# csiro-robotics/syropod_highlevel_controller

Measured on AMD Instinct MI355X. Metric: control-cycles/sec (all legs IK-solved), higher is better.
Workload: dtype f64

## Files before the change

syropod_highlevel_controller_amd/csrc/shc_cycle.hpp:

```cpp
#pragma once

#include "../../include/shc_batch.h"
#include "shc_leg.hpp"

namespace shc {

enum : int { WS_STARTING = 0, WS_MOVING = 1, WS_STOPPING = 2, WS_STOPPED = 3 };
enum : int { SS_SWING = 0, SS_STANCE = 1, SS_FORCE_STANCE = 2, SS_FORCE_STOP = 3 };
enum : int { PS_POSING = 0, PS_STOP_POSING = 1, PS_POSING_COMPLETE = 2 };
enum : int { PM_NONE = 0, PM_SWING = 1, PM_STANCE = 2, PM_STOP = 3 };

constexpr int LW_ACP = 1 << 2, LW_CFS = 1 << 3, LW_PM_SHIFT = 4, LW_NEG = 1 << 6, LW_IKFAIL = 1 << 7, LW_PHASE_SHIFT = 8,
              LW_PHASE_MASK = 0xFFFFF, LW_ZBV = 1 << 28, LW_ATT = 1 << 29, LW_ROTDEF = 1 << 30,
              LW_TARGROT = int(1u << 31);
constexpr int RW_LACP_SHIFT = 2, RW_LCFS_SHIFT = 6, RW_RTDA = 1 << 10, RW_APS_SHIFT = 11;

constexpr int kMaxAutoPosers = 8;
constexpr int kSwingTable = 64;
enum : unsigned { DIRTY_WALK_PLANE = 1, DIRTY_MANUAL = 2, DIRTY_SWING_ORG = 4, DIRTY_STANCE_ORG = 8,
                  DIRTY_TARG_DIR = 16,
                  DIRTY_LAST = DIRTY_TARG_DIR };
enum : unsigned { RT_MANUAL_LIVE = 1, RT_TOUCHDOWN = 2, RT_EXTERNAL = 4, RT_MANUAL_LEGS = 8, RT_EFFORT_LIVE = 16, RT_SKIP_MARKED = 32, RT_POSE_MARKED = 64 };

enum : unsigned { F_MANUAL = 1, F_AUTO = 2, F_INCL = 4, F_IMU = 8, F_ADM = 16, F_TIPF = 32, F_ODOM = 64, F_DYN = 1u << 31,
// ... 118 lines not shown
};
SHC_HD double set_precision3(double v) { return round_to_int(v * 1000.0) / 1000.0; }
SHC_HD double stance_span_change_y(const double *table, int leg, double default_shift_z) {
  const double *t = table + leg * SpanTable::kStride;
  const int n = int(t[0]);
  const double target = set_precision3(default_shift_z);
  int lower = -1, upper = -1;
  for (int k = 0; k < n; ++k) {
    const double h = t[2 + 2 * k];
    if (h > target && (upper < 0 || h < t[2 + 2 * upper])) upper = k;
    if (h <= target && (lower < 0 || h > t[2 + 2 * lower])) lower = k;
  }
  if (lower < 0 || upper < 0) return 0.0;
  const double uh = set_precision3(t[2 + 2 * upper]), lh = set_precision3(t[2 + 2 * lower]);
  const double i = (target - lh) / (uh - lh);
  const double radius = t[3 + 2 * lower] * (1.0 - i) + t[3 + 2 * upper] * i;
  return radius * t[1];
}

#if defined(__HIPCC__)

template <int L, int NJ, unsigned F>
constexpr bool phase_fences() {
#if defined(SHC_FENCE)
  return true;
#else
  constexpr bool exact = (F & (0x80000000u  | 0x40000000u )) == 0;
  constexpr bool octo_tipf = L == 8 && NJ == 5 && (F & 32u ) != 0 && (F & 16u ) == 0;
  return exact && ((NJ == 4 && (L == 4 || L == 8)) || octo_tipf);
#endif
}
#define SHC_PHASE_FENCE() do { if constexpr (phase_fences<L, NJ, F>()) __builtin_amdgcn_sched_barrier(0); } while (0)
#if defined(SHC_RES2_TIMING) && !defined(SHC_RES2_BUSY_ONLY)
__shared__ long long shc_ticks_lds[96];
__shared__ long long shc_acc_lds[96];
#define SHC_TICK(i) do { __builtin_amdgcn_sched_barrier(0); if (blockIdx.x == 1 && (threadIdx.x & 127) == 0) shc_ticks_lds[(threadIdx.x >> 7) * 32 + (i)] = __builtin_readcyclecounter(); __builtin_amdgcn_sched_barrier(0); } while (0)
#else
#define SHC_TICK(i) do {} while (0)
#endif
#ifdef SHC_ABLATE
#define SHC_DBG(P) ((P).debug_skip)
#else
#define SHC_DBG(P) 0
#endif
__device__ __forceinline__ int uni(int v) { return __builtin_amdgcn_readfirstlane(v); }

template <unsigned F>
struct Feat {
  __device__ __forceinline__ static bool manual(const CycleParams &P) { return (F & F_DYN) ? P.manual_posing != 0 : (F & F_MANUAL) != 0; }
  __device__ __forceinline__ static bool autop(const CycleParams &P) { return (F & F_DYN) ? P.auto_posing != 0 : (F & F_AUTO) != 0; }
  __device__ __forceinline__ static bool incl(const CycleParams &P) { return (F & F_DYN) ? P.inclination_posing != 0 : (F & F_INCL) != 0; }
  __device__ __forceinline__ static bool imu(const CycleParams &P) { return (F & F_DYN) ? P.imu_posing != 0 : (F & F_IMU) != 0; }
  __device__ __forceinline__ static bool adm(const CycleParams &P) { return (F & F_DYN) ? P.admittance_control != 0 : (F & F_ADM) != 0; }
  __device__ __forceinline__ static bool tipf(const CycleParams &P) { return (F & F_DYN) ? P.tip_force != 0 : (F & F_TIPF) != 0; }
  __device__ __forceinline__ static bool odom(const CycleParams &P) { return (F & F_DYN) ? P.odometry != 0 : (F & F_ODOM) != 0; }
};

template <int L>
struct Group {
  int base;
  __device__ __forceinline__ int get(int v, int j) const { return __shfl(v, base + j, 64); }
  __device__ __forceinline__ double get(double v, int j) const { return __shfl(v, base + j, 64); }
  __device__ __forceinline__ double sum(double v) const {
    double s = 0.0;
#pragma unroll
    for (int j = 0; j < L; ++j) s += get(v, j);
    return s;
  }
// ... 1444 lines not shown
```

syropod_highlevel_controller_amd/csrc/shc_cycle_inst.hip:

```cpp
#include "shc_cycle_kernel.hpp"
#include "shc_cycle_select.hpp"

#if !defined(SHC_INST_L) || !defined(SHC_INST_NJ) || !defined(SHC_INST_PART)
#error "compile with -DSHC_INST_L=<legs> -DSHC_INST_NJ=<joints> -DSHC_INST_PART=<0|1>"
#endif

#include <cstdio>
#include <cstdlib>
#include <mutex>
#include <set>
#include <tuple>

namespace shc {

static void note_kernel(const char *form, int legs, int joints, unsigned features) {
  static const char *path = std::getenv("SHC_KERNEL_LOG");
  if (!path) return;
  static std::mutex mu;
  static std::set<std::tuple<const char *, unsigned>> seen;
  std::lock_guard<std::mutex> lock(mu);
  if (!seen.insert({form, features}).second) return;
  if (FILE *f = std::fopen(path, "a")) {
    std::fprintf(f, "%s %d %d %u\n", form, legs, joints, features);
    std::fclose(f);
  }
}

template <int L, int NJ, unsigned F>
static void launch_cycle(const CycleLaunch &a) {
  constexpr int RPW = 64 / L;
  constexpr size_t wave_bytes = size_t(RobotFields::COUNT * RPW + PK_COUNT * 64 + (RobotFields::I_COUNT * RPW + 1) / 2) * 8;
#if SHC_INST_PART == 1
  if (a.fit) {
    a.fit->supported = has_resident(F) ? 1 : 0;
    a.fit->batch = has_batch(F) ? 1 : 0;
    a.fit->two_wave = has_two_wave(F) ? 1 : 0;
    a.fit->helper_wave = has_helper_wave(L, NJ, F) ? 1 : 0;
    a.fit->blocks_per_cu = 0;
    if constexpr (has_resident(F)) {
      int blocks = 0;
      if (hipOccupancyMaxActiveBlocksPerMultiprocessor(&blocks, shc_resident_kernel<L, NJ, F>, 64, wave_bytes) != hipSuccess) blocks = 0;
      a.fit->blocks_per_cu = blocks;
    }
  } else if (a.resident->batch_cycles != 0) {
    if constexpr (has_batch(F)) {
      note_kernel("batch", L, NJ, F);
      shc_batch_kernel<L, NJ, F><<<dim3(a.grid), dim3(a.block), wave_bytes * (a.block / 64), a.stream>>>(a.st, (const SharedConsts<L, NJ> *)a.consts, *a.resident, a.rt_flags);
    }
  } else if (a.block == 384) {
    if constexpr (has_helper_wave(L, NJ, F)) {
      static_assert(has_two_wave(F), "the three-role form is a form of the two-wavefront pipeline");
      note_kernel("resident3", L, NJ, F);
      shc_resident2_kernel<L, NJ, F, true><<<dim3(a.grid), dim3(384), 2 * wave_bytes + sizeof(Resident3Lds<L, NJ>), a.stream>>>(
          a.st, (const SharedConsts<L, NJ> *)a.consts, *a.resident, a.rt_flags);
    }
  } else if (a.block == 256) {
    if constexpr (has_two_wave(F)) {
      note_kernel("resident2", L, NJ, F);
      shc_resident2_kernel<L, NJ, F><<<dim3(a.grid), dim3(256), 2 * wave_bytes + sizeof(Resident2Lds<L, NJ>), a.stream>>>(
          a.st, (const SharedConsts<L, NJ> *)a.consts, *a.resident, a.rt_flags);
    }
  } else {
    if constexpr (has_resident(F)) {
      note_kernel("resident", L, NJ, F);
      shc_resident_kernel<L, NJ, F><<<dim3(a.grid), dim3(64), wave_bytes, a.stream>>>(a.st, (const SharedConsts<L, NJ> *)a.consts, *a.resident, a.rt_flags);
    }
  }
#else
  if constexpr (has_half_kernels(F)) {
    const int64_t waves = int64_t(a.grid) * (a.block / 64);
    if (a.half_steps >= 0 && (a.half_steps > 0 || waves >= 2048)) {
      note_kernel("half", L, NJ, F);
      for (int c = 0; c < a.n_cycles; ++c) {
        shc_cycle_half_kernel<L, NJ, F, ROLE_FRONT><<<dim3(a.grid), dim3(a.block), wave_bytes * (a.block / 64), a.stream>>>(
            a.st, (const SharedConsts<L, NJ> *)a.consts, a.rt_flags, a.wave0);
        shc_cycle_half_kernel<L, NJ, F, ROLE_BACK><<<dim3(a.grid), dim3(a.block), wave_bytes * (a.block / 64), a.stream>>>(
            a.st, (const SharedConsts<L, NJ> *)a.consts, a.rt_flags, a.wave0);
      }
      return;
    }
  }
  note_kernel("cycle", L, NJ, F);
  shc_cycle_kernel<L, NJ, F><<<dim3(a.grid), dim3(a.block), wave_bytes * (a.block / 64), a.stream>>>(a.st, (const SharedConsts<L, NJ> *)a.consts, a.n_cycles,
                                                                                              a.rt_flags, a.wave0);
#endif
}
// ... 22 lines not shown
```

syropod_highlevel_controller_amd/csrc/shc_cycle_kernel.hpp:

```cpp
#pragma once

#include "shc_cycle.hpp"
#include "shc_cycle_launch.hpp"

#include <hip/hip_runtime.h>

#include <type_traits>

namespace shc {

#ifndef SHC_WAVES_PER_SIMD
#define SHC_WAVES_PER_SIMD 2
#endif
#ifndef SHC_ROT_WAVES_PER_SIMD
#define SHC_ROT_WAVES_PER_SIMD 1
#endif
#ifndef SHC_TERRAIN_WAVES_PER_SIMD
#define SHC_TERRAIN_WAVES_PER_SIMD 2
#endif

struct LegPlanes {
  double2 *base;
  int64_t ns;
  uint32_t slot;
// ... 900 lines not shown
      if (t0 == 0) t0 = now;
      else if (now - t0 > 1000 * ticks_per_ms) {
        *fault = true;
        return true;
      }
    }
    return false;
  }
  __device__ __forceinline__ void operator()() const {
    volatile unsigned *flag = flag_at;
    unsigned spins = 0;
    u64 t0 = 0;
    while (*flag != want)
      if (give_up(spins, t0)) break;
    __builtin_amdgcn_fence(__ATOMIC_ACQUIRE, "workgroup");
  }
};
template <int L, int NJ>
struct Resident2Lds {
  double mailbox[2][2][13][64];
  double pose_c[2][2][64];
  unsigned pose_done[2];
  unsigned model_dirty[2], model_seen[2], model_fault[2];
  double stiff[2][64];
  int ikfail[2][64];
  unsigned long long ctrl[4][4];
};
template <int L, int NJ>
struct Resident3Lds : Resident2Lds<L, NJ> {
  int leg_word[2][2][64];
  unsigned back_seen[2];
  double tip_xy[2][2][2][64];
  unsigned front_done[2];
};

template <int L, int NJ, unsigned F, bool HELPER = false>
__global__ void __launch_bounds__(HELPER ? 384 : 256, 1) shc_resident2_kernel(DevState st, const SharedConsts<L, NJ> *gc, ResidentArgs A, unsigned rt_flags) {
  using R = RobotFields;
  using FD = Fields<NJ>;
  using FT = Feat<F>;
  constexpr int RPW = 64 / L;
  constexpr int kThreads = HELPER ? 384 : 256;
  if (blockIdx.x == 0) {
    if (threadIdx.x < 64) resident_relay<PART_GATE>(A);
    else if (threadIdx.x < 128) resident_relay<PART_DONE>(A);
    return;
  }
  __shared__ SharedConsts<L, NJ> C;
  extern __shared__ double wave_lds[];
  constexpr int kWaveDoubles = R::COUNT * RPW + PK_COUNT * 64 + (R::I_COUNT * RPW + 1) / 2;
  using Lds = std::conditional_t<HELPER, Resident3Lds<L, NJ>, Resident2Lds<L, NJ>>;
  Lds &X = *reinterpret_cast<Lds *>(wave_lds + 2 * kWaveDoubles);
  const bool manual_live = (rt_flags & RT_MANUAL_LIVE) != 0;
  const int lane = threadIdx.x & 63;
  const int wib = __builtin_amdgcn_readfirstlane(threadIdx.x >> 6);
  const int pair = wib & 1;
  const bool walker = wib < 2, helper = HELPER && wib >= 4, leader = wib == (HELPER ? 4 : 2);
  const int64_t wave = (int64_t(blockIdx.x) - 1) * 2 + pair;
  const bool active = wave < A.n_waves;
  const int64_t rob0 = wave * RPW;
  const int64_t left = st.n_robots - rob0;
  const int robots_here = !active ? 0 : (left < RPW ? (left < 0 ? 0 : int(left)) : RPW);
  int grp = lane / L;
  const int leg = lane - grp * L;
  const bool live = grp < robots_here;
  if (grp >= robots_here) grp = robots_here > 0 ? robots_here - 1 : 0;
  const uint32_t slot = uint32_t((active ? wave : 0) * 64 + grp * L + leg);
  double *const my_lds = wave_lds + pair * kWaveDoubles;
  Park pk{my_lds + R::COUNT * RPW, lane};
  double *tile = my_lds;
  int32_t *tile_i = reinterpret_cast<int32_t *>(my_lds + R::COUNT * RPW + PK_COUNT * 64);
  double *gtile = st.robd + (active ? wave : 0) * (R::COUNT * RPW);
  int32_t *gtile_i = st.robi + (active ? wave : 0) * (R::I_COUNT * RPW);
  const CycleParams &GP = gc->P;
  LegRegs<NJ> s;
  {
    using SC = SharedConsts<L, NJ>;
    constexpr int n16_all = sizeof(SC) / 16;
    constexpr int n16_core = (offsetof(SC, P) + offsetof(CycleParams, ap_start)) / 16;
    const int n16 = FT::autop(GP) ? n16_all : n16_core;
    const double2 *src = reinterpret_cast<const double2 *>(gc);
    double2 *dst = reinterpret_cast<double2 *>(&C);
    for (int i = threadIdx.x; i < n16; i += kThreads) dst[i] = src[i];
  }
  LegLoad<NJ> ll;
  if (active) {
    if (walker) {
      load_leg_issue<NJ, F, ROLE_FRONT>(ll, st, GP, slot);
      for (int i = lane; i < R::COUNT * RPW; i += 64) tile[i] = gtile[i];
      for (int i = lane; i < R::I_COUNT * RPW; i += 64) tile_i[i] = gtile_i[i];
// ... 33 lines not shown
  }
  unsigned dirty = 0;
  ResidentHeld held;
  const int swing_c_count_u = uni(P.swing_c_count);
  const auto publish_for_pose = [&](unsigned cycle, bool planes) {
    if (planes) {
      const V3 pp = rb.get3(R::PLANE_PREV), pn = rb.get3(R::PNORM_PREV);
#pragma unroll
      for (int par = 0; par < 2; ++par) {
        double *mb = &X.mailbox[pair][par][0][lane];
        mb[7 * 64] = pp.x, mb[8 * 64] = pp.y, mb[9 * 64] = pp.z, mb[10 * 64] = pn.x, mb[11 * 64] = pn.y, mb[12 * 64] = pn.z;
      }
    }
    if constexpr (HELPER) {
      X.leg_word[pair][cycle & 1][lane] = s.word;
      X.tip_xy[pair][cycle & 1][0][lane] = s.tip.x, X.tip_xy[pair][cycle & 1][1][lane] = s.tip.y;
    }
    else X.pose_c[pair][cycle & 1][lane] = walk_plane_control_candidate<L, NJ>(s.word, C, P, swing_c_count_u);
  };
  if (POSE_SPLIT && walker && active) publish_for_pose(0, true);
  const int64_t ns = st.n_slots;
  const unsigned out_slot_bytes = unsigned(NJ * ns * 16);
  const __amdgpu_buffer_rsrc_t out_rsrc = __builtin_amdgcn_make_buffer_rsrc(A.out, 0, int(unsigned(A.depth) * out_slot_bytes), 0x00020000);
  const u64 emergency_ticks = 4 * A.idle_ticks + 2000 * A.ticks_per_ms;
  unsigned k = 0, c_front = 0, c_back = 0, oslot = 0;
  bool prev_real = false;
  u64 prev_h0 = 0, prev_h1 = 0;
  u64 gate_pref = leader ? ld_agent(&A.ctl->gate) : 0;
  u64 bubble_since = 0;
  FrontToBack fb{V3{1, 0, 0}, false, LS_WALKING};
  fb.uf = load_uni_flags(C.P);
  OdomCache odom_cache;
  Pose owpp_cache = pose_identity();
  const bool poser = HELPER ? helper : !walker;
  if (POSE_SPLIT && active && poser) owpp_cache = rb.getpose(R::OWPP);
  constexpr bool ODOM_REGS = NJ <= 3;
  constexpr bool ODOM_WALKER = NJ > 3 || (F & (F_ADM | F_IMU | F_INCL | F_AUTO | F_DYN)) != 0;
  static_assert(!HELPER || (POSE_SPLIT && !ODOM_WALKER && ODOM_REGS), "the helper takes the pose and the odometry off the MODEL wavefront");
  const bool odom_mine = ODOM_WALKER ? walker : poser;
  double odom[4] = {0.0, 0.0, 1.0, 0.0};
  if (ODOM_REGS && FT::odom(P) && active && odom_mine) {
#pragma unroll
    for (int i = 0; i < 4; ++i) odom[i] = rb.get(R::ODOM + i);
  }
#ifdef SHC_RES2_TIMING
  long long tm_busy = 0, tm_total0 = __builtin_readcyclecounter(), tm_real = 0;
#ifndef SHC_RES2_BUSY_ONLY
  if (threadIdx.x < 96) shc_acc_lds[threadIdx.x] = 0;
#endif
#endif
#ifdef SHC_RES2_TIMING
#define SHC_R2_ITER_BEGIN() const long long tm0 = __builtin_readcyclecounter(); SHC_TICK(19)
#ifndef SHC_RES2_BUSY_ONLY
#define SHC_R2_PHASES(THREAD, ...)                                                                                                  \
  if (kind == IT_REAL && prev_real && blockIdx.x == 1 && threadIdx.x == (THREAD)) {       \
    const int base = ((THREAD) >> 7) * 32;                                                                                         \
    const int order[] = {__VA_ARGS__};                                                                                             \
    for (int i = 1; i < int(sizeof(order) / sizeof(int)); ++i) shc_acc_lds[base + order[i]] += shc_ticks_lds[base + order[i]] - shc_ticks_lds[base + order[i - 1]]; \
  }
#else
#define SHC_R2_PHASES(THREAD, ...)
#endif
#define SHC_R2_ITER_END(THREAD, ...)                                                         \
  if (kind == IT_REAL && prev_real) tm_busy += __builtin_readcyclecounter() - tm0, ++tm_real; \
  SHC_R2_PHASES(THREAD, __VA_ARGS__)
#else
#define SHC_R2_ITER_BEGIN() do {} while (0)
#define SHC_R2_ITER_END(THREAD, ...) do {} while (0)
#endif
  LegInRing<NJ> in_at;
  int in_src_force = -1000, in_src_effort = -1000;
  const auto leader_decide = [&](const int kind, int &nk, u64 &nh0v, u64 &nh1v) __attribute__((always_inline)) {
    u64 gate;
    if (kind == IT_BUBBLE) {
      __builtin_amdgcn_s_sleep(2);
      gate = uni64(ld_agent(&A.ctl->gate));
    } else {
      gate = uni64(gate_pref);
    }
    const unsigned db = unsigned(gate), sp = unsigned(gate >> 32);
    const unsigned cn = c_front + (kind == IT_REAL ? 1u : 0u);
// ... 114 lines not shown
        }
#ifdef SHC_ABLATE
        if (!(P.debug_skip & 65536))
#endif
        if (POSE_SPLIT) publish_for_pose(c_front + 1, fb.plane_prev_changed);
        SHC_TICK(29);
        double *mb = &X.mailbox[pair][c_front & 1][0][lane];
        mb[0] = out.poser_tip.x, mb[64] = out.poser_tip.y, mb[128] = out.poser_tip.z;
        if constexpr (ODOM_WALKER) {
          if (FT::odom(P) && __any(fb.odom_run)) {
            if (fb.odom_run) {
              if constexpr (ODOM_REGS) odometry_advance(odom[0], odom[1], odom[2], odom[3], P, fb.odom_vel.x, fb.odom_vel.y, fb.odom_vel.z, &odom_cache);
              else odometry_step(rb, P, fb.odom_vel.x, fb.odom_vel.y, fb.odom_vel.z, &odom_cache);
            }
          }
        } else if (FT::odom(P)) {
          mb[192] = fb.odom_vel.x, mb[256] = fb.odom_vel.y, mb[320] = fb.odom_vel.z, mb[384] = fb.odom_run ? 1.0 : 0.0;
        }
        SHC_TICK(22);
      }
      SHC_TICK(23);
      if (kind == IT_EXIT) break;
      if constexpr (HELPER) {
        SHC_R2_ITER_END(kWalkerThread, 19, 20, 21, 2, 3, 4, 6, 7, 18, 16, 8, 17, 15, 29, 22, 23);
      } else {
        SHC_R2_ITER_END(kWalkerThread, 19, 20, 21, 2, 3, 4, 5, 6, 7, 16, 8, 17, 15, 29, 22, 23);
      }
      if (kind == IT_REAL) ++c_front;
      prev_real = kind == IT_REAL;
      __syncthreads();
      ++k;
    }
  } else if (helper) {
    if constexpr (HELPER) for (;;) {
      SHC_R2_ITER_BEGIN();
      const int kind = __builtin_amdgcn_readfirstlane(int(X.ctrl[k & 3][0]));
      const u64 h0 = uni64(X.ctrl[k & 3][1]), h1 = uni64(X.ctrl[k & 3][2]);
      SHC_TICK(29);
      int nk = IT_EXIT;
      u64 nh0v = 0, nh1v = 0;
      if (leader && kind != IT_EXIT) leader_decide(kind, nk, nh0v, nh1v);
      if (active) {
        SHC_TICK(24);
        if (kind == IT_REAL) front_of_cycle(h0, h1);
        SHC_TICK(1);
        if (kind == IT_REAL) pose_of_cycle(h0, h1);
        SHC_TICK(25);
        if (prev_real) {
          if (FT::odom(P)) odometry_of_cycle(&X.mailbox[pair][c_back & 1][0][lane]);
          ++c_back;
        }
        SHC_TICK(26);
      }
      if (leader && kind != IT_EXIT && lane == 0) leader_announce(nk, nh0v, nh1v);
      SHC_TICK(14);
      if (kind == IT_EXIT) break;
      SHC_R2_ITER_END(256, 19, 29, 24, 1, 30, 25, 26, 14);
      if (kind == IT_REAL) ++c_front;
      prev_real = kind == IT_REAL;
      __syncthreads();
      ++k;
    }
  } else {
    for (;;) {
      SHC_R2_ITER_BEGIN();
      const int kind = __builtin_amdgcn_readfirstlane(int(X.ctrl[k & 3][0]));
      const u64 h0 = uni64(X.ctrl[k & 3][1]), h1 = uni64(X.ctrl[k & 3][2]);
      SHC_TICK(29);
      [[maybe_unused]] int nk = IT_EXIT;
      [[maybe_unused]] u64 nh0v = 0, nh1v = 0;
      if constexpr (!HELPER) if (leader && kind != IT_EXIT) leader_decide(kind, nk, nh0v, nh1v);
      if (active) {
        SHC_TICK(24);
        if constexpr (POSE_SPLIT && !HELPER) if (kind == IT_REAL) pose_of_cycle(h0, h1);
        SHC_TICK(25);
        if (prev_real) {
          resident_take_inputs<RPW, ROBOT_NONE, true>(A, c_back, prev_h0, prev_h1, wave, lane, tile, tile_i, dirty, held, st.n_robots);
          if (held.src_force != in_src_force || held.src_effort != in_src_effort) {
            in_at = leg_inputs_in_force<L, NJ>(A, st.legd, held.src_force, held.src_effort, ns, slot, wave * RPW + grp, leg);
            in_src_force = held.src_force, in_src_effort = held.src_effort;
          }
          LegInRing<NJ> in = in_at;
          if (FT::tipf(P)) in.prefetch_effort();
          SHC_TICK(31);
          const double *mb = &X.mailbox[pair][c_back & 1][0][lane];
          out.poser_tip = V3{mb[0], mb[64], mb[128]};
          if constexpr (!ODOM_WALKER && !HELPER) if (FT::odom(P)) odometry_of_cycle(mb);
          out.adm_delta = V3{0, 0, 0};
          if (FT::adm(P)) cycle_admittance<NJ>(s, out, P, in);
          s.word = 0;
          SHC_TICK(26);
          cycle_back<L, NJ, F>(s, out, C, leg, st.legd, ns, slot, nullptr, in, fb);
          SHC_TICK(27);
          asm volatile("s_waitcnt vmcnt(0)" ::: "memory");
// ... 12 lines not shown
#pragma unroll
              for (int p = 0; p < NJ; ++p) {
                const u64 a = u64(__double_as_longlong(flat[2 * p])), b = u64(__double_as_longlong(flat[2 * p + 1]));
                const v4u w = {unsigned(a), unsigned(a >> 32), unsigned(b), unsigned(b >> 32)};
                __builtin_amdgcn_raw_buffer_store_b128(w, out_rsrc, unsigned((int64_t(p) * ns + slot) * 16), soff, 16 );
              }
            }
          }
          ++c_back;
          oslot = oslot + 1 == unsigned(A.depth) ? 0 : oslot + 1;
          SHC_TICK(28);
        }
        if (kind != IT_REAL) {
          asm volatile("s_waitcnt vmcnt(0)" ::: "memory");
          if (lane == 0) st_agent(A.progress + wave, u64(c_back));
        }
      }
      if constexpr (!HELPER) if (leader && kind != IT_EXIT && lane == 0) leader_announce(nk, nh0v, nh1v);
      SHC_TICK(14);
      if (kind == IT_EXIT) break;
      SHC_R2_ITER_END(kModelThread, 19, 29, 24, 30, 25, 31, 26, 9, 10, 11, 12, 27, 13, 28, 14);
      if (kind == IT_REAL) ++c_front;
      prev_real = kind == IT_REAL;
      prev_h0 = h0, prev_h1 = h1;
      __syncthreads();
      ++k;
    }
  }
#undef SHC_R2_ITER_BEGIN
#undef SHC_R2_ITER_END
#undef SHC_R2_PHASES
#ifdef SHC_RES2_TIMING
  if (blockIdx.x == 1 && lane == 0 && pair == 0) {
    unsigned long long *rec = reinterpret_cast<unsigned long long *>(A.ctl) + 8, *dbg = rec + (walker ? 0 : helper ? 72 : 4);
    dbg[0] = tm_busy, dbg[1] = tm_real, dbg[2] = __builtin_readcyclecounter() - tm_total0, dbg[3] = k;
#ifndef SHC_RES2_BUSY_ONLY
    const int from = int(threadIdx.x >> 7) * 32, to = walker ? 8 : helper ? 80 : 40;
    for (int i = 0; i < 32; ++i) rec[to + i] = (unsigned long long)shc_acc_lds[from + i];
#endif
  }
#endif
  if (active && ODOM_REGS && FT::odom(P) && odom_mine) {
#pragma unroll
    for (int i = 0; i < 4; ++i) rb.put(R::ODOM + i, odom[i]);
  }
  if (active) {
    if (walker) {
      X.stiff[pair][lane] = s.stiff;
    } else {
      if (!helper) X.ikfail[pair][lane] = s.word & LW_IKFAIL;
      if constexpr (HELPER) if (!helper && lane == 0) X.back_seen[pair] = held.seen;
      if (poser) {
        if (POSE_SPLIT) {
          unsigned d = 0;
#pragma unroll
          for (unsigned b = 1; b <= DIRTY_LAST; b <<= 1)
            if (__any((dirty & b) != 0)) d |= b;
          if (lane == 0) X.model_dirty[pair] = d, X.model_seen[pair] = held.seen;
        }
        if (lane == 0) X.model_fault[pair] = held.fault ? 1u : 0u;
      }
    }
  }
  __syncthreads();
  if (!active || helper) return;
  if (walker) {
    if (POSE_SPLIT) dirty |= X.model_dirty[pair], held.seen |= X.model_seen[pair];
    if constexpr (HELPER) held.seen |= X.back_seen[pair];
    if (X.model_fault[pair]) held.fault = true;
    if (c_front > 0) s.word = (s.word & ~LW_IKFAIL) | X.ikfail[pair][lane];
    {
      unsigned d = 0;
#pragma unroll
      for (unsigned b = 1; b <= DIRTY_LAST; b <<= 1)
        if (__any((dirty & b) != 0)) d |= b;
      dirty = d;
    }
    if (live) store_leg<NJ, F, ROLE_FRONT>(s, out, pk, st, P, slot, dirty);
    __builtin_amdgcn_wave_barrier();
    store_rob_fields<RPW, 0, R::PLANE>(tile, gtile, lane);
    if (dirty & DIRTY_WALK_PLANE) store_rob_fields<RPW, R::PLANE, R::VIN>(tile, gtile, lane);
    if (FT::manual(P) && manual_live && (dirty & DIRTY_MANUAL)) store_rob_fields<RPW, R::MPOSE, R::MANUAL_END>(tile, gtile, lane);
    if (FT::imu(P)) store_rob_fields<RPW, R::ABSE, R::GYRO>(tile, gtile, lane);
    if (FT::incl(P) && FT::autop(P)) store_rob_fields<RPW, R::APREV, R::APREV_END>(tile, gtile, lane);
    store_rob_fields<RPW, R::CPOSE, R::CPOSE_END>(tile, gtile, lane);
    if (FT::odom(P)) store_rob_fields<RPW, R::ODOM, R::ODOM_END>(tile, gtile, lane);
    if (lane < (R::I_POSE_PHASE + 1) * RPW) gtile_i[lane] = tile_i[lane];
    store_rob_fields<RPW, R::VIN, R::CORE_END>(tile, gtile, lane);
    if (held.seen & (1u << RG_IMU)) {
      store_rob_fields<RPW, R::GYRO, R::IMU_END>(tile, gtile, lane);
      store_rob_fields<RPW, R::IMUQ, R::IMUQ_END>(tile, gtile, lane);
    }
    if ((held.seen & (1u << RG_RESET)) && lane < RPW) gtile_i[R::I_RESET_MODE * RPW + lane] = tile_i[R::I_RESET_MODE * RPW + lane];
    if (lane == 0) {
      if (held.fault) __hip_atomic_fetch_or(&A.ctl->fault, 1ull, __ATOMIC_RELAXED, __HIP_MEMORY_SCOPE_AGENT);
      __hip_atomic_fetch_add(&A.ctl->exited, 1ull, __ATOMIC_RELAXED, __HIP_MEMORY_SCOPE_AGENT);
    }
  } else {
    s.stiff = X.stiff[pair][lane];
    if (live) {
      store_leg<NJ, F, ROLE_BACK>(s, out, pk, st, P, slot, 0);
      carry_leg_inputs<L, NJ>(A, st, held, ns, slot, leg);
// ... 6 lines not shown
```

syropod_highlevel_controller_amd/csrc/shc_cycle_launch.hpp:

```cpp
#pragma once

#include "shc_cycle.hpp"

#include <hip/hip_runtime.h>

namespace shc {

enum : int { RG_VEL = 0, RG_IMU = 1, RG_POSE = 2, RG_RESET = 3, RG_FORCE = 4, RG_EFFORT = 5, RG_COUNT = 6 };
enum : int { RIN_VEL = 0, RIN_IMU = 3, RIN_POSE = 10, RIN_COUNT = 16 };

constexpr int kResidentHeaders = 1024;
constexpr int kBoundSets = 4;
enum : int { BND_LIN = 0, BND_ANG = 1, BND_IMUQ = 2, BND_IMUW = 3, BND_FORCE = 4, BND_EFFORT = 5, BND_COUNT = 6 };
constexpr unsigned kResidentDirect = 1u << 15;
struct ResidentCtl {
  unsigned long long gate;
  unsigned long long exited;
  unsigned long long fault;
  unsigned long long pad[5];
  unsigned long long dbg[112];
};
struct ResidentHost {
  unsigned long long doorbell;
  unsigned long long stop;
  unsigned long long done;
  unsigned long long exited;
  unsigned long long heartbeat;
  unsigned long long fault;
  unsigned long long late_reads;
  unsigned long long pad_[1];
  unsigned long long records[kResidentHeaders * 2];
};
struct ResidentHeader {
  unsigned long long tag;
  unsigned short mask;
  unsigned char pos[RG_COUNT];
};
static_assert(sizeof(ResidentHeader) == 16, "header is read as two 8-byte words");
enum : unsigned long long { RESIDENT_EXIT_STOP = 1, RESIDENT_EXIT_IDLE = 2, RESIDENT_EXIT_MAX = 3, RESIDENT_EXIT_FAULT = 4 };

struct ResidentArgs {
  ResidentCtl *ctl;
  ResidentHost *host;
  unsigned long long *progress;
  ResidentHeader *headers;
  const double *bound[kBoundSets][BND_COUNT];
  const double *rin;
  const int32_t *rini;
  const double *force;
  const double *effort;
  double *out;
  int depth;
  unsigned max_cycles;
// ... 40 lines not shown
```

syropod_highlevel_controller_amd/csrc/shc_resident.hpp:

```cpp

struct Resident {
  bool active = false;
  int depth = 0;
  ResidentArgs args{};
  ResidentHost *host = nullptr;
  ResidentHost *host_dev = nullptr;
  ResidentCtl *ctl = nullptr;
  unsigned long long *progress = nullptr;
  ResidentHeader *headers = nullptr;
  double *rin = nullptr, *force = nullptr, *effort = nullptr, *out = nullptr, *stage = nullptr;
  int32_t *rini = nullptr;
  size_t stage_bytes = 0;
  static constexpr int kPinSlots = 4;
  unsigned *post_blocks_done = nullptr;
  char *pin = nullptr, *pin_dev = nullptr;
  hipEvent_t pin_ev[kPinSlots] = {};
  unsigned long long pin_uses = 0;
  hipStream_t in_stream = nullptr;
  hipStream_t loop_stream = nullptr;
  hipEvent_t loop_ev = nullptr;
  unsigned long long published = 0;
  unsigned long long posted = 0;
  unsigned long long posts[RG_COUNT] = {};
  std::vector<unsigned long long> post_cycle[RG_COUNT];
  unsigned max_cycles = 0;
  unsigned long long wall_khz = 100000;
  bool poisoned = false;
  bool stream_doorbell_pending = false;
  unsigned groups_posted = 0;
  bool two_wave = false;
  bool helper_wave = false;
  long long direct_last = -1;
  hipEvent_t rows_ev[2] = {};
  long long read_queued = -1;
};

__global__ void resident_doorbell_kernel(ResidentHost *host, unsigned long long value) {
  __hip_atomic_store(&host->doorbell, value, __ATOMIC_RELAXED, __HIP_MEMORY_SCOPE_SYSTEM);
}

struct ResidentPostSlot {
  int pos[RG_COUNT];
  unsigned mask;
  unsigned long long cycle;
  unsigned long long doorbell;
  ResidentHost *host;
  unsigned *blocks_done;
};
struct ResidentPost : ResidentPostSlot {
  const double *lin, *ang, *imu_q, *imu_w, *tvi, *rvi, *force, *effort;
  const int32_t *reset;
};
__device__ __forceinline__ void resident_put(double *p, double v) {
  __hip_atomic_store(reinterpret_cast<unsigned long long *>(p), (unsigned long long)__double_as_longlong(v), __ATOMIC_RELAXED, __HIP_MEMORY_SCOPE_AGENT);
}
__device__ __forceinline__ void resident_post_header(const ResidentPostSlot &pp, ResidentHeader *headers) {
  unsigned long long h1 = pp.mask & 0xffffu;
  for (int gi = 0; gi < RG_COUNT; ++gi) h1 |= (unsigned long long)(pp.pos[gi] & 0xff) << (16 + 8 * gi);
  unsigned long long *hp = reinterpret_cast<unsigned long long *>(headers + (pp.cycle & (kResidentHeaders - 1)));
  __hip_atomic_store(hp + 1, h1, __ATOMIC_RELAXED, __HIP_MEMORY_SCOPE_AGENT);
  __hip_atomic_store(hp, pp.cycle + 1, __ATOMIC_RELAXED, __HIP_MEMORY_SCOPE_AGENT);
}
__device__ __forceinline__ void resident_post_doorbell(const ResidentPostSlot &pp) {
  if (pp.doorbell == 0) return;
// ... 226 lines not shown
  r->direct_last = -1;
  r->read_queued = -1;
  r->groups_posted = 0;
  r->stream_doorbell_pending = false;
  for (int gi = 0; gi < RG_COUNT; ++gi) {
    r->posts[gi] = 0;
    std::fill(r->post_cycle[gi].begin(), r->post_cycle[gi].end(), 0ull);
  }
  r->max_cycles = unsigned(max_cycles);
  ResidentArgs &A = r->args;
  A.ctl = r->ctl;
  A.host = r->host_dev;
  A.progress = r->progress;
  A.headers = r->headers;
  memcpy(A.bound, e->bound_inputs, sizeof A.bound);
  A.rin = r->rin;
  A.rini = r->rini;
  A.force = r->force;
  A.effort = r->effort;
  A.out = r->out;
  A.depth = ring_depth;
  A.max_cycles = r->max_cycles;
  int wall_khz = 0;
  if (hipDeviceGetAttribute(&wall_khz, hipDeviceAttributeWallClockRate, e->device) != hipSuccess || wall_khz <= 0) wall_khz = 100000;
  r->wall_khz = (unsigned long long)wall_khz;
  A.idle_ticks = (unsigned long long)(idle_timeout_ms ? idle_timeout_ms : 5000) * r->wall_khz;
  A.ticks_per_ms = r->wall_khz;
  A.n_waves = e->n_waves;
  A.touchdown_threshold = e->params.touchdown_threshold;
  A.liftoff_threshold = e->params.liftoff_threshold;
  e->plan_poser_tips_current = false;
  const bool two_wave = fit.two_wave && !(e->features & SHC_FEAT_RESIDENT_ONE_WAVE) && (e->n_waves + 1) / 2 + 1 <= prop.multiProcessorCount;
  r->two_wave = two_wave;
  const char *two_role = getenv("SHC_RESIDENT_TWO_ROLE");
  r->helper_wave = two_wave && fit.helper_wave && !(two_role && atoi(two_role) > 0);
  HIP_TRY(hipEventRecord(r->loop_ev, e->stream));
  HIP_TRY(hipStreamWaitEvent(r->loop_stream, r->loop_ev, 0));
  CycleLaunch a = cycle_launch(e);
  a.stream = r->loop_stream, a.resident = &A;
  a.grid = two_wave ? unsigned((e->n_waves + 1) / 2 + 1) : unsigned(e->n_waves + 1), a.block = r->helper_wave ? 384 : two_wave ? 256 : 64;
  {
    const int rc = launch_cycle_for(e, a);
    if (rc != SHC_OK) return rc;
  }
  HIP_TRY(hipGetLastError());
  r->active = true;
  return SHC_OK;
}

static int resident_wait_direct_installed(Resident *r) {
  if (r->direct_last < 0) return SHC_OK;
  const unsigned long long need = (unsigned long long)r->direct_last + 1;
  if (!spin_until([&] { return host_load(&r->host->done) >= need || host_load(&r->host->exited) != 0; }, 5.0))
    return fail(SHC_ERR_TIMEOUT, "resident mode: a direct post is still waiting to run");
  r->direct_last = -1;
  return SHC_OK;
}

static int resident_alive(Resident *r) {
  if (const unsigned long long why = host_load(&r->host->exited))
    return fail(SHC_ERR_TIMEOUT, std::string("resident mode: the device loop has stopped by itself (") +
                                     (why == RESIDENT_EXIT_IDLE ? "idle timeout" : why == RESIDENT_EXIT_MAX ? "max_cycles" : why == RESIDENT_EXIT_FAULT ? "fault" : "stop") +
                                     " after " + std::to_string(host_load(&r->host->done)) + " cycles): call shc_engine_resident_end");
  return SHC_OK;
}

constexpr double kResidentPostPatience = 5.0;
static int resident_post_admit(shc_engine *e, unsigned mask, unsigned long long &c) {
  Resident *r = e->res;
  if ((mask & ((1u << RG_POSE) | (1u << RG_RESET))) && !(e->rt_flags & RT_MANUAL_LIVE))
    return fail(SHC_ERR_UNSUPPORTED, "pose inputs: give the engine one (shc_engine_set_pose_input / set_pose_reset_mode) before shc_engine_resident_begin");
  if ((mask & (1u << RG_EFFORT)) && !(e->rt_flags & RT_EFFORT_LIVE))
    return fail(SHC_ERR_UNSUPPORTED, "joint efforts: give the engine one (shc_engine_set_joint_effort) before shc_engine_resident_begin");
// ... 233 lines not shown
  if (rc != SHC_OK) return rc;
  Resident *r = e->res;
  const bool active = r && r->active;
  if (published) *published = active ? int64_t(r->published) : 0;
  if (completed) *completed = active ? int64_t(host_load(&r->host->done)) : 0;
  if (running) *running = active && host_load(&r->host->exited) == 0 ? 1 : 0;
  return SHC_OK;
}

extern "C" int shc_engine_resident_end(shc_engine *e, int64_t *cycles_run) {
  int rc = resident_require(e, true);
  if (rc != SHC_OK) return rc;
  Resident *r = e->res;
  HIP_TRY(hipSetDevice(e->device));
  HIP_TRY(hipStreamSynchronize(r->in_stream));
  const int direct_rc = resident_wait_direct_installed(r);
  const std::string direct_msg = direct_rc != SHC_OK ? std::string(shc_last_error()) : std::string();
  if (direct_rc == SHC_OK) host_store(&r->host->doorbell, r->published);
  host_store(&r->host->stop, direct_rc == SHC_OK ? r->published : 0ull);
  const bool answered = spin_until([&] { return host_load(&r->host->exited) != 0; }, r->poisoned ? 5.0 : 30.0);
  if (!answered) {
    r->poisoned = true;
    return fail(SHC_ERR_TIMEOUT, "resident mode: the device loop did not answer the stop request in time; the engine stays in resident mode - call "
                                 "shc_engine_resident_end again");
  }
  hipError_t err = hipStreamSynchronize(r->loop_stream);
  if (err == hipSuccess) err = hipStreamSynchronize(e->stream);
  r->active = false;
  r->poisoned = false;
#ifdef SHC_RES2_TIMING
  if (err == hipSuccess) {
    ResidentCtl c;
    (void)hipMemcpy(&c, r->ctl, sizeof c, hipMemcpyDeviceToHost);
    for (int w = 0; w < (r->helper_wave ? 3 : 2); ++w) {
      const unsigned long long *b = c.dbg + (w == 2 ? 72 : 4 * w);
      fprintf(stderr, "[res2 timing] %s: %.0f clocks busy per steady REAL iteration (%llu of them), loop %llu clocks, %llu iterations\n", w == 0 ? "walker" : w == 1 ? "model " : "helper",
              b[1] ? double(b[0]) / double(b[1]) : 0.0, b[1], b[2], b[3]);
    }
#ifndef SHC_RES2_BUSY_ONLY
    const int order[] = {20, 21, 2, 3, 4, 5, 6, 7, 16, 8, 17, 15, 29, 22, 23};
    const char *wname[] = {"control words (LDS) read", "inputs of the cycle taken", "cycle_front entry", "robot word / command read, stop predicates", "(pose elsewhere)", "getLimit",
                           "velocity shaping", "walk state machine", "stepper (stride, Bezier, tip)", "tip rotation / iteratePhase / planes / leg word", "wait for the pose flag",
                           "pose read + updateStance", "control input for the next pose published", "mailbox written", "to the barrier"};
    const double its = c.dbg[1] ? double(c.dbg[1]) : 1.0;
    fprintf(stderr, "[res2 timing] walker of pair 0, mean clocks per phase:\n");
    for (int i = 0; i < int(sizeof(order) / sizeof(int)); ++i) {
      if (r->helper_wave && order[i] == 5) continue;
      if (r->helper_wave && order[i] == 16) fprintf(stderr, "[res2 timing]   walker t%-2d %-58s %7.0f\n", 18, "stepper, first half + wait for the front", double(c.dbg[8 + 18]) / its);
      fprintf(stderr, "[res2 timing]   walker t%-2d %-58s %7.0f\n", order[i], r->helper_wave && order[i] == 6 ? "command predicate" : wname[i], double(c.dbg[8 + order[i]]) / its);
    }
    const int morder[] = {29, 24, 30, 25, 31, 26, 9, 10, 11, 12, 27, 13, 28, 14};
    const char *mname[] = {"control words (LDS) read", "leader: gate, what the next iteration is, header prefetch issued", "pose inputs of the cycle taken",
                           "updateCurrentPose of the walker's cycle + flag", "leg inputs in force, joint efforts prefetched", "mailbox read, odometry, admittance",
                           "cycle_back entry (desired tip)", "IK step + joint update", "sin / cos, chain, Jacobian", "model tip, tip force", "cycle_back exit",
                           "wait for the previous stores + progress word", "output-ring stores issued", "control words written (leader: waits for its loads)"};
    const double mits = c.dbg[5] ? double(c.dbg[5]) : 1.0;
    fprintf(stderr, "[res2 timing] model wavefront of pair 0 (the leader), mean clocks per phase:\n");
    for (int i = 0; i < int(sizeof(morder) / sizeof(int)); ++i) {
      if (r->helper_wave && (morder[i] == 30 || morder[i] == 25)) continue;
      fprintf(stderr, "[res2 timing]   model  t%-2d %-58s %7.0f\n", morder[i], mname[i], double(c.dbg[40 + morder[i]]) / mits);
    }
    if (r->helper_wave) {
      const int horder[] = {29, 24, 1, 30, 25, 26, 14};
      const char *hname[] = {"control words (LDS) read", "leader: gate, what the next iteration is, header prefetch issued", "front: command, getLimit, velocity shaping + flag", "pose inputs of the cycle taken",
                             "leg words reduced, updateCurrentPose of the walker's cycle + flag", "odometry", "control words written (leader: waits for its loads)"};
      const double hits = c.dbg[73] ? double(c.dbg[73]) : 1.0;
      fprintf(stderr, "[res2 timing] helper wavefront of pair 0 (the leader), mean clocks per phase:\n");
      for (int i = 0; i < int(sizeof(horder) / sizeof(int)); ++i) fprintf(stderr, "[res2 timing]   helper t%-2d %-58s %7.0f\n", horder[i], hname[i], double(c.dbg[80 + horder[i]]) / hits);
    }
#endif
  }
#endif
  const unsigned long long reason = host_load(&r->host->exited), done = host_load(&r->host->done);
  if (cycles_run) *cycles_run = int64_t(done);
  if (r->groups_posted & (1u << RG_FORCE)) e->rt_flags |= RT_TOUCHDOWN;
  if (err != hipSuccess) return fail(SHC_ERR_HIP, std::string("hipStreamSynchronize: ") + hipGetErrorString(err));
  if (direct_rc != SHC_OK) return fail(direct_rc, direct_msg + " (the loop was stopped after " + std::to_string(done) + " cycles)");
  if (reason == RESIDENT_EXIT_FAULT || host_load(&r->host->fault) != 0)
    return fail(SHC_ERR_HIP, "resident mode: a wavefront gave up waiting for the relay; restore the engine from a snapshot");
  if (host_load(&r->host->late_reads) != 0)
    return fail(SHC_ERR_TIMEOUT, "resident mode: a stream-ordered read (shc_engine_resident_get_joint_state_async) gave up waiting for its cycle");
  if (!((reason == RESIDENT_EXIT_STOP || reason == RESIDENT_EXIT_MAX) && done == r->published))
    return fail(SHC_ERR_TIMEOUT, std::string("resident mode: the device loop had stopped by itself (") +
                                     (reason == RESIDENT_EXIT_IDLE ? "idle timeout" : reason == RESIDENT_EXIT_MAX ? "max_cycles" : "unknown") + ") after " +
                                     std::to_string(done) + " of " + std::to_string(r->published) + " published cycles");
  return SHC_OK;
}

static int step_k_out_ring(shc_engine *e, int K) {
  const size_t need = size_t(K) * size_t(e->NJ) * size_t(e->n_slots) * 16;
  if (e->k_out && e->k_out_bytes >= need) return SHC_OK;
  if (e->k_out) {
    const int rc = join_side(e);
    if (rc != SHC_OK) return rc;
    HIP_TRY(hipStreamSynchronize(e->stream));
    (void)hipFree(e->k_out);
    e->k_out = nullptr, e->k_out_bytes = 0;
  }
  HIP_TRY(hipMalloc(reinterpret_cast<void **>(&e->k_out), need));
  e->k_out_bytes = need;
  return SHC_OK;
// ... 115 lines not shown
```

Baseline: 1.783 billion.

## Split the helper role into separate front and pose helper wavefronts

```diff
diff --git a/syropod_highlevel_controller_amd/csrc/shc_cycle.hpp b/syropod_highlevel_controller_amd/csrc/shc_cycle.hpp
--- a/syropod_highlevel_controller_amd/csrc/shc_cycle.hpp
+++ b/syropod_highlevel_controller_amd/csrc/shc_cycle.hpp
@@ -174,8 +174,8 @@
 }
 #define SHC_PHASE_FENCE() do { if constexpr (phase_fences<L, NJ, F>()) __builtin_amdgcn_sched_barrier(0); } while (0)
 #if defined(SHC_RES2_TIMING) && !defined(SHC_RES2_BUSY_ONLY)
-__shared__ long long shc_ticks_lds[96];
-__shared__ long long shc_acc_lds[96];
+__shared__ long long shc_ticks_lds[128];
+__shared__ long long shc_acc_lds[128];
 #define SHC_TICK(i) do { __builtin_amdgcn_sched_barrier(0); if (blockIdx.x == 1 && (threadIdx.x & 127) == 0) shc_ticks_lds[(threadIdx.x >> 7) * 32 + (i)] = __builtin_readcyclecounter(); __builtin_amdgcn_sched_barrier(0); } while (0)
 #else
 #define SHC_TICK(i) do {} while (0)
diff --git a/syropod_highlevel_controller_amd/csrc/shc_cycle_inst.hip b/syropod_highlevel_controller_amd/csrc/shc_cycle_inst.hip
--- a/syropod_highlevel_controller_amd/csrc/shc_cycle_inst.hip
+++ b/syropod_highlevel_controller_amd/csrc/shc_cycle_inst.hip
@@ -47,11 +47,17 @@
       note_kernel("batch", L, NJ, F);
       shc_batch_kernel<L, NJ, F><<<dim3(a.grid), dim3(a.block), wave_bytes * (a.block / 64), a.stream>>>(a.st, (const SharedConsts<L, NJ> *)a.consts, *a.resident, a.rt_flags);
     }
+  } else if (a.block == 512) {
+    if constexpr (has_helper_wave(L, NJ, F)) {
+      static_assert(has_two_wave(F), "the helper forms are forms of the two-wavefront pipeline");
+      note_kernel("resident3", L, NJ, F);
+      shc_resident2_kernel<L, NJ, F, 2><<<dim3(a.grid), dim3(512), 2 * wave_bytes + sizeof(Resident3Lds<L, NJ>), a.stream>>>(
+          a.st, (const SharedConsts<L, NJ> *)a.consts, *a.resident, a.rt_flags);
+    }
   } else if (a.block == 384) {
     if constexpr (has_helper_wave(L, NJ, F)) {
-      static_assert(has_two_wave(F), "the three-role form is a form of the two-wavefront pipeline");
-      note_kernel("resident3", L, NJ, F);
-      shc_resident2_kernel<L, NJ, F, true><<<dim3(a.grid), dim3(384), 2 * wave_bytes + sizeof(Resident3Lds<L, NJ>), a.stream>>>(
+      note_kernel("resident3_one_helper", L, NJ, F);
+      shc_resident2_kernel<L, NJ, F, 1><<<dim3(a.grid), dim3(384), 2 * wave_bytes + sizeof(Resident3Lds<L, NJ>), a.stream>>>(
           a.st, (const SharedConsts<L, NJ> *)a.consts, *a.resident, a.rt_flags);
     }
   } else if (a.block == 256) {
diff --git a/syropod_highlevel_controller_amd/csrc/shc_cycle_kernel.hpp b/syropod_highlevel_controller_amd/csrc/shc_cycle_kernel.hpp
--- a/syropod_highlevel_controller_amd/csrc/shc_cycle_kernel.hpp
+++ b/syropod_highlevel_controller_amd/csrc/shc_cycle_kernel.hpp
@@ -956,15 +956,17 @@
   unsigned back_seen[2];
   double tip_xy[2][2][2][64];
   unsigned front_done[2];
+  unsigned front_dirty[2], front_seen[2], front_fault[2];
 };
 
-template <int L, int NJ, unsigned F, bool HELPER = false>
-__global__ void __launch_bounds__(HELPER ? 384 : 256, 1) shc_resident2_kernel(DevState st, const SharedConsts<L, NJ> *gc, ResidentArgs A, unsigned rt_flags) {
+template <int L, int NJ, unsigned F, int HELPERS = 0>
+__global__ void __launch_bounds__(256 + 128 * HELPERS, 1) shc_resident2_kernel(DevState st, const SharedConsts<L, NJ> *gc, ResidentArgs A, unsigned rt_flags) {
   using R = RobotFields;
   using FD = Fields<NJ>;
   using FT = Feat<F>;
   constexpr int RPW = 64 / L;
-  constexpr int kThreads = HELPER ? 384 : 256;
+  constexpr bool HELPER = HELPERS > 0, FOUR = HELPERS == 2;
+  constexpr int kThreads = 256 + 128 * HELPERS;
   if (blockIdx.x == 0) {
     if (threadIdx.x < 64) resident_relay<PART_GATE>(A);
     else if (threadIdx.x < 128) resident_relay<PART_DONE>(A);
@@ -980,6 +982,7 @@
   const int wib = __builtin_amdgcn_readfirstlane(threadIdx.x >> 6);
   const int pair = wib & 1;
   const bool walker = wib < 2, helper = HELPER && wib >= 4, leader = wib == (HELPER ? 4 : 2);
+  const bool fronter = FOUR ? wib >= 6 : helper;
   const int64_t wave = (int64_t(blockIdx.x) - 1) * 2 + pair;
   const bool active = wave < A.n_waves;
   const int64_t rob0 = wave * RPW;
@@ -1079,7 +1082,7 @@
   fb.uf = load_uni_flags(C.P);
   OdomCache odom_cache;
   Pose owpp_cache = pose_identity();
-  const bool poser = HELPER ? helper : !walker;
+  const bool poser = HELPER ? helper && !(FOUR && fronter) : !walker;
   if (POSE_SPLIT && active && poser) owpp_cache = rb.getpose(R::OWPP);
   constexpr bool ODOM_REGS = NJ <= 3;
   constexpr bool ODOM_WALKER = NJ > 3 || (F & (F_ADM | F_IMU | F_INCL | F_AUTO | F_DYN)) != 0;
@@ -1093,7 +1096,7 @@
 #ifdef SHC_RES2_TIMING
   long long tm_busy = 0, tm_total0 = __builtin_readcyclecounter(), tm_real = 0;
 #ifndef SHC_RES2_BUSY_ONLY
-  if (threadIdx.x < 96) shc_acc_lds[threadIdx.x] = 0;
+  if (threadIdx.x < 128) shc_acc_lds[threadIdx.x] = 0;
 #endif
 #endif
 #ifdef SHC_RES2_TIMING
@@ -1274,34 +1277,52 @@
       ++k;
     }
   } else if (helper) {
-    if constexpr (HELPER) for (;;) {
-      SHC_R2_ITER_BEGIN();
-      const int kind = __builtin_amdgcn_readfirstlane(int(X.ctrl[k & 3][0]));
-      const u64 h0 = uni64(X.ctrl[k & 3][1]), h1 = uni64(X.ctrl[k & 3][2]);
-      SHC_TICK(29);
-      int nk = IT_EXIT;
-      u64 nh0v = 0, nh1v = 0;
-      if (leader && kind != IT_EXIT) leader_decide(kind, nk, nh0v, nh1v);
-      if (active) {
+    const auto helper_loop = [&](auto with_front, auto with_rest) __attribute__((always_inline)) {
+      constexpr bool FRONT = decltype(with_front)::value, REST = decltype(with_rest)::value;
+      constexpr int kThread = FOUR && FRONT ? 384 : 256;
+      for (;;) {
+        SHC_R2_ITER_BEGIN();
+        const int kind = __builtin_amdgcn_readfirstlane(int(X.ctrl[k & 3][0]));
+        const u64 h0 = uni64(X.ctrl[k & 3][1]), h1 = uni64(X.ctrl[k & 3][2]);
+        SHC_TICK(29);
+        [[maybe_unused]] int nk = IT_EXIT;
+        [[maybe_unused]] u64 nh0v = 0, nh1v = 0;
+        if constexpr (REST && !FOUR) if (leader && kind != IT_EXIT) leader_decide(kind, nk, nh0v, nh1v);
         SHC_TICK(24);
-        if (kind == IT_REAL) front_of_cycle(h0, h1);
-        SHC_TICK(1);
-        if (kind == IT_REAL) pose_of_cycle(h0, h1);
-        SHC_TICK(25);
-        if (prev_real) {
-          if (FT::odom(P)) odometry_of_cycle(&X.mailbox[pair][c_back & 1][0][lane]);
-          ++c_back;
-        }
-        SHC_TICK(26);
-      }
-      if (leader && kind != IT_EXIT && lane == 0) leader_announce(nk, nh0v, nh1v);
-      SHC_TICK(14);
-      if (kind == IT_EXIT) break;
-      SHC_R2_ITER_END(256, 19, 29, 24, 1, 30, 25, 26, 14);
-      if (kind == IT_REAL) ++c_front;
-      prev_real = kind == IT_REAL;
-      __syncthreads();
-      ++k;
+        if (active) {
+          if constexpr (FRONT) if (kind == IT_REAL) front_of_cycle(h0, h1);
+          SHC_TICK(1);
+          if constexpr (REST) {
+            if (kind == IT_REAL) pose_of_cycle(h0, h1);
+            SHC_TICK(25);
+            if constexpr (FOUR) if (leader && kind != IT_EXIT) leader_decide(kind, nk, nh0v, nh1v);
+            SHC_TICK(2);
+            if (prev_real) {
+              if (FT::odom(P)) odometry_of_cycle(&X.mailbox[pair][c_back & 1][0][lane]);
+              ++c_back;
+            }
+            SHC_TICK(26);
+          }
+        }
+        if constexpr (REST) if (leader && kind != IT_EXIT && lane == 0) leader_announce(nk, nh0v, nh1v);
+        SHC_TICK(14);
+        if (kind == IT_EXIT) break;
+        if constexpr (REST) {
+          SHC_R2_ITER_END(kThread, 19, 29, 24, 1, 30, 25, 2, 26, 14);
+        } else {
+          SHC_R2_ITER_END(kThread, 19, 29, 24, 1, 14);
+        }
+        if (kind == IT_REAL) ++c_front;
+        prev_real = kind == IT_REAL;
+        __syncthreads();
+        ++k;
+      }
+    };
+    if constexpr (FOUR) {
+      if (fronter) helper_loop(std::true_type{}, std::false_type{});
+      else helper_loop(std::false_type{}, std::true_type{});
+    } else if constexpr (HELPER) {
+      helper_loop(std::true_type{}, std::true_type{});
     }
   } else {
     for (;;) {
@@ -1380,10 +1401,11 @@
 #undef SHC_R2_PHASES
 #ifdef SHC_RES2_TIMING
   if (blockIdx.x == 1 && lane == 0 && pair == 0) {
-    unsigned long long *rec = reinterpret_cast<unsigned long long *>(A.ctl) + 8, *dbg = rec + (walker ? 0 : helper ? 72 : 4);
+    const bool second_helper = FOUR && fronter;
+    unsigned long long *rec = reinterpret_cast<unsigned long long *>(A.ctl) + 8, *dbg = rec + (walker ? 0 : second_helper ? 112 : helper ? 72 : 4);
     dbg[0] = tm_busy, dbg[1] = tm_real, dbg[2] = __builtin_readcyclecounter() - tm_total0, dbg[3] = k;
 #ifndef SHC_RES2_BUSY_ONLY
-    const int from = int(threadIdx.x >> 7) * 32, to = walker ? 8 : helper ? 80 : 40;
+    const int from = int(threadIdx.x >> 7) * 32, to = walker ? 8 : second_helper ? 120 : helper ? 80 : 40;
     for (int i = 0; i < 32; ++i) rec[to + i] = (unsigned long long)shc_acc_lds[from + i];
 #endif
   }
@@ -1408,6 +1430,13 @@
         }
         if (lane == 0) X.model_fault[pair] = held.fault ? 1u : 0u;
       }
+      if constexpr (FOUR) if (fronter) {
+        unsigned d = 0;
+#pragma unroll
+        for (unsigned b = 1; b <= DIRTY_LAST; b <<= 1)
+          if (__any((dirty & b) != 0)) d |= b;
+        if (lane == 0) X.front_dirty[pair] = d, X.front_seen[pair] = held.seen, X.front_fault[pair] = held.fault ? 1u : 0u;
+      }
     }
   }
   __syncthreads();
@@ -1416,6 +1445,10 @@
     if (POSE_SPLIT) dirty |= X.model_dirty[pair], held.seen |= X.model_seen[pair];
     if constexpr (HELPER) held.seen |= X.back_seen[pair];
     if (X.model_fault[pair]) held.fault = true;
+    if constexpr (FOUR) {
+      dirty |= X.front_dirty[pair], held.seen |= X.front_seen[pair];
+      if (X.front_fault[pair]) held.fault = true;
+    }
     if (c_front > 0) s.word = (s.word & ~LW_IKFAIL) | X.ikfail[pair][lane];
     {
       unsigned d = 0;
diff --git a/syropod_highlevel_controller_amd/csrc/shc_cycle_launch.hpp b/syropod_highlevel_controller_amd/csrc/shc_cycle_launch.hpp
--- a/syropod_highlevel_controller_amd/csrc/shc_cycle_launch.hpp
+++ b/syropod_highlevel_controller_amd/csrc/shc_cycle_launch.hpp
@@ -18,7 +18,7 @@
   unsigned long long exited;
   unsigned long long fault;
   unsigned long long pad[5];
-  unsigned long long dbg[112];
+  unsigned long long dbg[152];
 };
 struct ResidentHost {
   unsigned long long doorbell;
diff --git a/syropod_highlevel_controller_amd/csrc/shc_resident.hpp b/syropod_highlevel_controller_amd/csrc/shc_resident.hpp
--- a/syropod_highlevel_controller_amd/csrc/shc_resident.hpp
+++ b/syropod_highlevel_controller_amd/csrc/shc_resident.hpp
@@ -29,7 +29,7 @@
   bool stream_doorbell_pending = false;
   unsigned groups_posted = 0;
   bool two_wave = false;
-  bool helper_wave = false;
+  int helper_waves = 0;
   long long direct_last = -1;
   hipEvent_t rows_ev[2] = {};
   long long read_queued = -1;
@@ -322,13 +322,14 @@
   e->plan_poser_tips_current = false;
   const bool two_wave = fit.two_wave && !(e->features & SHC_FEAT_RESIDENT_ONE_WAVE) && (e->n_waves + 1) / 2 + 1 <= prop.multiProcessorCount;
   r->two_wave = two_wave;
-  const char *two_role = getenv("SHC_RESIDENT_TWO_ROLE");
-  r->helper_wave = two_wave && fit.helper_wave && !(two_role && atoi(two_role) > 0);
+  const char *two_role = getenv("SHC_RESIDENT_TWO_ROLE"), *three_role = getenv("SHC_RESIDENT_THREE_ROLE");
+  const bool room_for_four = (e->n_waves + 1) / 2 + 1 <= prop.multiProcessorCount - kXcds;
+  r->helper_waves = !(two_wave && fit.helper_wave) || (two_role && atoi(two_role) > 0) ? 0 : (three_role && atoi(three_role) > 0) || !room_for_four ? 1 : 2;
   HIP_TRY(hipEventRecord(r->loop_ev, e->stream));
   HIP_TRY(hipStreamWaitEvent(r->loop_stream, r->loop_ev, 0));
   CycleLaunch a = cycle_launch(e);
   a.stream = r->loop_stream, a.resident = &A;
-  a.grid = two_wave ? unsigned((e->n_waves + 1) / 2 + 1) : unsigned(e->n_waves + 1), a.block = r->helper_wave ? 384 : two_wave ? 256 : 64;
+  a.grid = two_wave ? unsigned((e->n_waves + 1) / 2 + 1) : unsigned(e->n_waves + 1), a.block = r->helper_waves ? 256 + 128 * r->helper_waves : two_wave ? 256 : 64;
   {
     const int rc = launch_cycle_for(e, a);
     if (rc != SHC_OK) return rc;
@@ -628,10 +629,11 @@
   if (err == hipSuccess) {
     ResidentCtl c;
     (void)hipMemcpy(&c, r->ctl, sizeof c, hipMemcpyDeviceToHost);
-    for (int w = 0; w < (r->helper_wave ? 3 : 2); ++w) {
-      const unsigned long long *b = c.dbg + (w == 2 ? 72 : 4 * w);
-      fprintf(stderr, "[res2 timing] %s: %.0f clocks busy per steady REAL iteration (%llu of them), loop %llu clocks, %llu iterations\n", w == 0 ? "walker" : w == 1 ? "model " : "helper",
-              b[1] ? double(b[0]) / double(b[1]) : 0.0, b[1], b[2], b[3]);
+    const bool helper_wave = r->helper_waves > 0;
+    for (int w = 0; w < 2 + r->helper_waves; ++w) {
+      const unsigned long long *b = c.dbg + (w == 3 ? 112 : w == 2 ? 72 : 4 * w);
+      fprintf(stderr, "[res2 timing] %s: %.0f clocks busy per steady REAL iteration (%llu of them), loop %llu clocks, %llu iterations\n",
+              w == 0 ? "walker" : w == 1 ? "model " : w == 3 ? "front helper" : r->helper_waves == 2 ? "pose helper" : "helper", b[1] ? double(b[0]) / double(b[1]) : 0.0, b[1], b[2], b[3]);
     }
 #ifndef SHC_RES2_BUSY_ONLY
     const int order[] = {20, 21, 2, 3, 4, 5, 6, 7, 16, 8, 17, 15, 29, 22, 23};
@@ -641,9 +643,9 @@
     const double its = c.dbg[1] ? double(c.dbg[1]) : 1.0;
     fprintf(stderr, "[res2 timing] walker of pair 0, mean clocks per phase:\n");
     for (int i = 0; i < int(sizeof(order) / sizeof(int)); ++i) {
-      if (r->helper_wave && order[i] == 5) continue;
-      if (r->helper_wave && order[i] == 16) fprintf(stderr, "[res2 timing]   walker t%-2d %-58s %7.0f\n", 18, "stepper, first half + wait for the front", double(c.dbg[8 + 18]) / its);
-      fprintf(stderr, "[res2 timing]   walker t%-2d %-58s %7.0f\n", order[i], r->helper_wave && order[i] == 6 ? "command predicate" : wname[i], double(c.dbg[8 + order[i]]) / its);
+      if (helper_wave && order[i] == 5) continue;
+      if (helper_wave && order[i] == 16) fprintf(stderr, "[res2 timing]   walker t%-2d %-58s %7.0f\n", 18, "stepper, first half + wait for the front", double(c.dbg[8 + 18]) / its);
+      fprintf(stderr, "[res2 timing]   walker t%-2d %-58s %7.0f\n", order[i], helper_wave && order[i] == 6 ? "command predicate" : wname[i], double(c.dbg[8 + order[i]]) / its);
     }
     const int morder[] = {29, 24, 30, 25, 31, 26, 9, 10, 11, 12, 27, 13, 28, 14};
     const char *mname[] = {"control words (LDS) read", "leader: gate, what the next iteration is, header prefetch issued", "pose inputs of the cycle taken",
@@ -653,16 +655,22 @@
     const double mits = c.dbg[5] ? double(c.dbg[5]) : 1.0;
     fprintf(stderr, "[res2 timing] model wavefront of pair 0 (the leader), mean clocks per phase:\n");
     for (int i = 0; i < int(sizeof(morder) / sizeof(int)); ++i) {
-      if (r->helper_wave && (morder[i] == 30 || morder[i] == 25)) continue;
+      if (helper_wave && (morder[i] == 30 || morder[i] == 25)) continue;
       fprintf(stderr, "[res2 timing]   model  t%-2d %-58s %7.0f\n", morder[i], mname[i], double(c.dbg[40 + morder[i]]) / mits);
     }
-    if (r->helper_wave) {
-      const int horder[] = {29, 24, 1, 30, 25, 26, 14};
+    for (int h = 0; h < r->helper_waves; ++h) {
+      const int horder[] = {29, 24, 1, 30, 25, 2, 26, 14};
       const char *hname[] = {"control words (LDS) read", "leader: gate, what the next iteration is, header prefetch issued", "front: command, getLimit, velocity shaping + flag", "pose inputs of the cycle taken",
-                             "leg words reduced, updateCurrentPose of the walker's cycle + flag", "odometry", "control words written (leader: waits for its loads)"};
-      const double hits = c.dbg[73] ? double(c.dbg[73]) : 1.0;
-      fprintf(stderr, "[res2 timing] helper wavefront of pair 0 (the leader), mean clocks per phase:\n");
-      for (int i = 0; i < int(sizeof(horder) / sizeof(int)); ++i) fprintf(stderr, "[res2 timing]   helper t%-2d %-58s %7.0f\n", horder[i], hname[i], double(c.dbg[80 + horder[i]]) / hits);
+                             "leg words reduced, updateCurrentPose of the walker's cycle + flag", "leader (four roles): gate, next iteration, header prefetch issued", "odometry",
+                             "control words written (leader: waits for its loads)"};
+      const int busy = h ? 112 : 72, phases = h ? 120 : 80;
+      const double hits = c.dbg[busy + 1] ? double(c.dbg[busy + 1]) : 1.0;
+      const char *who = r->helper_waves == 1 ? "helper" : h ? "front helper" : "pose helper";
+      fprintf(stderr, "[res2 timing] %s wavefront of pair 0%s, mean clocks per phase:\n", who, h == 0 ? " (the leader)" : "");
+      for (int i = 0; i < int(sizeof(horder) / sizeof(int)); ++i) {
+        if (h == 1 && (horder[i] == 30 || horder[i] == 25 || horder[i] == 2 || horder[i] == 26)) continue;
+        fprintf(stderr, "[res2 timing]   %s t%-2d %-58s %7.0f\n", who, horder[i], hname[i], double(c.dbg[phases + horder[i]]) / hits);
+      }
     }
 #endif
   }
```

After: 1.892 billion (median of 6 runs). +6.1%, better.
